# NeuralRevenant/RASSEngine

Hardware: AMD Instinct MI355X
Metric: queries/sec, exact cosine top-10 over N x 1024-d fp32 corpus in HBM (higher is better)
Workload: dtype f32; 1 GPU; 1000000 x 1024-d flat cosine top-10, 1 x MI355X, precomputed embeddings (BASELINE configs[1]); rows_per_gpu=1000000, rows_global=1000000, dim=1024, k=10, query_batch=32, corpus_dtype=f32, layout=tile16, mode=flat

## Files before the change

### include/rass_engine.h

```cpp
#ifndef RASS_ENGINE_H
#define RASS_ENGINE_H

#include <stddef.h>
#include <stdint.h>

#ifdef __cplusplus
extern "C" {
#endif

#define RASS_ABI_VERSION 1

typedef enum rass_status {
    RASS_OK = 0,
    RASS_ERR_INVALID = -1,
    RASS_ERR_HIP = -2,
    RASS_ERR_OOM = -3,
    RASS_ERR_NOT_FOUND = -4,
    RASS_ERR_UNSUPPORTED = -5,
    RASS_ERR_IO = -6
} rass_status;

typedef enum rass_dtype {
    RASS_F32 = 0,
    RASS_BF16 = 1,
// ... 183 lines not shown
                                     int64_t* d_out_ids, int64_t* d_n_buckets, int64_t* d_total_hits, int32_t* d_status);

int rass_index_rows_gram(rass_index_t* idx, const int64_t* rows, int n_lists, int list_len, float* out);
int rass_index_rows_gram_device(rass_index_t* idx, const int64_t* d_rows, int n_lists, int list_len, float* d_out);

int rass_index_search_mmr(rass_index_t* idx, const float* queries, int nq, int k, int fetch_k,
                          const float* lambda, const int32_t* q_filter, const int32_t* q_filter_mask,
                          float* out_scores, int64_t* out_ids, int32_t* out_rank);
int rass_index_search_mmr_device(rass_index_t* idx, const float* d_queries, int nq, int k, int fetch_k,
                                 const float* d_lambda, const int32_t* d_q_filter, const int32_t* d_q_filter_mask,
                                 int64_t id_base, float* d_out_scores, int64_t* d_out_ids, int32_t* d_out_rank);

#define RASS_PREFILTER_OFF 0
#define RASS_PREFILTER_BF16 1
#define RASS_PREFILTER_INT8 2
#define RASS_PREFILTER_INT8_EXACT 3
int rass_index_set_prefilter(rass_index_t* idx, int enable);
int rass_index_get_prefilter(const rass_index_t* idx);
int rass_index_certify_stats(rass_index_t* idx, int64_t* queries, int64_t* certified, int64_t* fallbacks, float* R, float* V);
int rass_index_candidates_exact_device(rass_index_t* idx, const float* d_queries, int nq, int k, const int32_t* d_q_filter,
                                       float* d_cand_scores, int64_t* d_cand_rows, float* d_tau, int32_t* d_certified);
int rass_index_sample_floor_device(rass_index_t* idx, const float* d_queries, int nq, int k, const int32_t* d_q_filter,
                                   int32_t* d_out_rows, float* d_out_scores);
int rass_index_candidates_device(rass_index_t* idx, const float* d_queries, int nq, const int32_t* d_q_filter,
                                 float* d_cand_scores, int64_t* d_cand_rows);

int rass_index_save(rass_index_t* idx, const char* path);
int rass_index_load(rass_engine_t* eng, const char* name, const char* path,
                    rass_index_t** out);

int rass_index_fill_synthetic(rass_index_t* idx, int64_t n, uint64_t seed,
                              int64_t row_id_base);


size_t rass_scan_workspace_bytes(int nq, int k);

int rass_pack_rows_f32(const float* d_in, int64_t in_stride, float* d_packed,
                       int64_t row_stride, int64_t first_row, int64_t n, int dim,
                       int normalize, void* stream);
int rass_unpack_rows_f32(const float* d_packed, int64_t row_stride,
                         int64_t first_row, int64_t n, int dim, float* d_out,
                         int64_t out_stride, void* stream);
int rass_gather_rows_f32(const float* d_packed, int64_t row_stride, int64_t n_rows,
                         const int64_t* d_row_ids, int64_t n, int dim, float* d_out,
                         int64_t out_stride, void* stream);
int rass_compact_plan(const int32_t* d_tags, int64_t n_rows, int64_t* d_new_row,
// ... 203 lines not shown
```

### rassengine_amd/_native.py

```python
from __future__ import annotations

import ctypes
import os
from typing import Optional

_HERE = os.path.dirname(os.path.abspath(__file__))
LIB_PATH = os.environ.get("RASS_HIP_LIB") or os.path.join(_HERE, "lib", "librass_hip.so")

RASS_OK = 0
RASS_MAX_K = 32
RASS_MAX_K_MULTIPASS = 4096
RASS_TAG_PATIENT_MASK = 0x00FFFFFF
RASS_TAG_DOCTYPE_SHIFT = 24
RASS_TAG_DOCTYPE_MASK = 0x7F000000
RASS_MAX_QBATCH = 32
RASS_MAX_DEVICE_BATCH = 4096
RASS_MAX_MMR_FETCH = 128
RASS_F32 = 0
RASS_BF16 = 1
RASS_QFILTER_NONE = -1
RASS_MAX_ATTRS = 8
RASS_ATTR_MISSING = -(1 << 31)
RASS_MAX_ATTR_CLAUSES = 64
RASS_ATTR_ALL, RASS_ATTR_ANY = 0, 1
# ... 103 lines not shown
    "rass_index_search_grouped_keys_device": (ctypes.c_int, [ctypes.c_void_p, ctypes.c_void_p, ctypes.c_int, ctypes.c_int, ctypes.c_void_p, ctypes.c_int64, ctypes.c_int32, ctypes.c_void_p, ctypes.c_int, ctypes.c_int64, ctypes.c_void_p, ctypes.c_void_p, ctypes.c_int64, ctypes.c_void_p, ctypes.c_void_p, ctypes.c_void_p, ctypes.c_void_p, ctypes.c_void_p]),
    "rass_index_aggregate_keys": (ctypes.c_int, [ctypes.c_void_p, ctypes.c_void_p, ctypes.c_int, ctypes.c_void_p, ctypes.c_int, ctypes.c_void_p, ctypes.c_int64, ctypes.c_int32, ctypes.c_void_p, ctypes.c_int, ctypes.c_int64, ctypes.c_void_p, ctypes.c_void_p, ctypes.c_void_p, ctypes.c_void_p, ctypes.c_void_p, ctypes.c_void_p, ctypes.c_void_p, ctypes.c_void_p]),
    "rass_index_aggregate_keys_device": (ctypes.c_int, [ctypes.c_void_p, ctypes.c_void_p, ctypes.c_int, ctypes.c_void_p, ctypes.c_int, ctypes.c_void_p, ctypes.c_int64, ctypes.c_int32, ctypes.c_void_p, ctypes.c_int, ctypes.c_int64, ctypes.c_void_p, ctypes.c_void_p, ctypes.c_int64, ctypes.c_void_p, ctypes.c_void_p, ctypes.c_void_p, ctypes.c_void_p, ctypes.c_void_p, ctypes.c_void_p, ctypes.c_void_p]),
    "rass_index_rows_gram": (ctypes.c_int, [ctypes.c_void_p, ctypes.c_void_p, ctypes.c_int, ctypes.c_int, ctypes.c_void_p]),
    "rass_index_rows_gram_device": (ctypes.c_int, [ctypes.c_void_p, ctypes.c_void_p, ctypes.c_int, ctypes.c_int,
                                                   ctypes.c_void_p]),
    "rass_index_search_mmr": (ctypes.c_int, [ctypes.c_void_p, ctypes.c_void_p, ctypes.c_int, ctypes.c_int, ctypes.c_int,
                                             ctypes.c_void_p, ctypes.c_void_p, ctypes.c_void_p, ctypes.c_void_p, ctypes.c_void_p,
                                             ctypes.c_void_p]),
    "rass_index_search_mmr_device": (ctypes.c_int, [ctypes.c_void_p, ctypes.c_void_p, ctypes.c_int, ctypes.c_int, ctypes.c_int,
                                                    ctypes.c_void_p, ctypes.c_void_p, ctypes.c_void_p, ctypes.c_int64,
                                                    ctypes.c_void_p, ctypes.c_void_p, ctypes.c_void_p]),
    "rass_index_set_prefilter": (ctypes.c_int, [ctypes.c_void_p, ctypes.c_int]),
    "rass_index_get_prefilter": (ctypes.c_int, [ctypes.c_void_p]),
    "rass_index_candidates_device": (ctypes.c_int, [ctypes.c_void_p, ctypes.c_void_p, ctypes.c_int, ctypes.c_void_p,
                                                    ctypes.c_void_p, ctypes.c_void_p]),
    "rass_index_certify_stats": (ctypes.c_int, [ctypes.c_void_p, ctypes.c_void_p, ctypes.c_void_p, ctypes.c_void_p,
                                                ctypes.c_void_p, ctypes.c_void_p]),
    "rass_index_candidates_exact_device": (ctypes.c_int, [ctypes.c_void_p, ctypes.c_void_p, ctypes.c_int, ctypes.c_int,
                                                          ctypes.c_void_p, ctypes.c_void_p, ctypes.c_void_p, ctypes.c_void_p,
                                                          ctypes.c_void_p]),
    "rass_index_sample_floor_device": (ctypes.c_int, [ctypes.c_void_p, ctypes.c_void_p, ctypes.c_int, ctypes.c_int,
                                                      ctypes.c_void_p, ctypes.c_void_p, ctypes.c_void_p]),
    "rass_index_save": (ctypes.c_int, [ctypes.c_void_p, ctypes.c_char_p]),
    "rass_index_load": (ctypes.c_int, [ctypes.c_void_p, ctypes.c_char_p, ctypes.c_char_p, c_void_pp]),
    "rass_index_fill_synthetic": (ctypes.c_int, [ctypes.c_void_p, ctypes.c_int64, ctypes.c_uint64,
                                                 ctypes.c_int64]),
    "rass_scan_workspace_bytes": (ctypes.c_size_t, [ctypes.c_int, ctypes.c_int]),
    "rass_scan_topk_f32": (ctypes.c_int, [ctypes.c_void_p, ctypes.c_int64, ctypes.c_int, ctypes.c_int64,
                                          ctypes.c_void_p, ctypes.c_void_p, ctypes.c_int, ctypes.c_void_p,
                                          ctypes.c_int, ctypes.c_int64, ctypes.c_void_p, ctypes.c_void_p,
                                          ctypes.c_void_p, ctypes.c_size_t, ctypes.c_void_p]),
    "rass_pack_rows_f32": (ctypes.c_int, [ctypes.c_void_p, ctypes.c_int64, ctypes.c_void_p, ctypes.c_int64,
                                          ctypes.c_int64, ctypes.c_int64, ctypes.c_int, ctypes.c_int,
                                          ctypes.c_void_p]),
    "rass_unpack_rows_f32": (ctypes.c_int, [ctypes.c_void_p, ctypes.c_int64, ctypes.c_int64, ctypes.c_int64,
                                            ctypes.c_int, ctypes.c_void_p, ctypes.c_int64, ctypes.c_void_p]),
    "rass_gather_rows_f32": (ctypes.c_int, [ctypes.c_void_p, ctypes.c_int64, ctypes.c_int64, ctypes.c_void_p, ctypes.c_int64,
                                            ctypes.c_int, ctypes.c_void_p, ctypes.c_int64, ctypes.c_void_p]),
    "rass_compact_plan": (ctypes.c_int, [ctypes.c_void_p, ctypes.c_int64, ctypes.c_void_p, ctypes.c_void_p, ctypes.c_void_p,
                                         ctypes.c_void_p, ctypes.c_size_t, ctypes.c_void_p]),
    "rass_compact_plan_workspace_bytes": (ctypes.c_size_t, [ctypes.c_int64]),
    "rass_compact_rows_f32": (ctypes.c_int, [ctypes.c_void_p, ctypes.c_void_p, ctypes.c_int64, ctypes.c_void_p, ctypes.c_int64,
                                             ctypes.c_int64, ctypes.c_void_p]),
    "rass_topk_merge": (ctypes.c_int, [ctypes.c_void_p, ctypes.c_void_p, ctypes.c_int, ctypes.c_int, ctypes.c_int,
                                       ctypes.c_void_p, ctypes.c_void_p, ctypes.c_void_p]),
# ... 167 lines not shown
```

### rassengine_amd/csrc/api_internal.h

```cpp
#pragma once

#include <hip/hip_runtime.h>
#include <stdint.h>
#include <stdio.h>
#include <stdlib.h>
#include <string.h>
#include <unistd.h>

#include <algorithm>
#include <atomic>
#include <condition_variable>
#include <map>
#include <mutex>
#include <new>
#include <string>
#include <type_traits>
#include <vector>

#include "../../include/rass_engine.h"
#include "kernels.h"

namespace rass {
namespace host {

// ... 76 lines not shown
struct ScratchView {
    float* q_padded;
    float* part_scores;
    int64_t* part_ids;
    unsigned short* q_bf16;
    float* cand_scores;
    int64_t* cand_ids;
    float* sample_best;
    size_t total;
};
ScratchView scratch_layout(unsigned char* base, int nq, int k);

struct BatchView {
    float* q_padded;
    float* part_scores;
    int64_t* part_ids;
    float* sample_best;
    unsigned char* q_small;
    float* cand_scores;
    int64_t* cand_rows;
    unsigned char* rep_qfrag;
    unsigned char* rep_part;
    int* rep_row;
    size_t total;
    size_t part_per_group;
    float* group_sample(int g) const { return sample_best + (int64_t)g * 32 * rass::kMaxSampleGroups; }
};
BatchView batch_layout(unsigned char* base, int groups, int grid, int k, int64_t stride, bool candidates = false);

struct CertView {
    float* q_padded;
    signed char* q8;
    rass::CertQInfo* qinfo;
    float* sample;
    float* list_s;
    int32_t* list_r;
    int32_t* list_n;
    float* list_floor;
    int64_t* cand_rows;
    float* rr_s;
    int64_t* rr_i;
    float* tau;
    int32_t *fail_idx, *fail_flag, *fail_n;
    float* fb_q;
    int32_t *fb_filter, *fb_mask;
    float* fb_s;
// ... 186 lines not shown
    float* d_pair_scores = nullptr;
    int64_t* d_pair_ids = nullptr;
    unsigned char* d_batch = nullptr;
    size_t batch_bytes = 0;
    unsigned char* d_allow_ws = nullptr;
    size_t allow_ws_bytes = 0;
};

namespace rass {
namespace host {

int set_device(const rass_engine* eng);
int index_reserve(rass_index* idx, int64_t need_rows);
void index_free_slabs(rass_index* idx);
int index_attr_ensure(rass_index* idx, int col);
int index_refresh_copies(rass_index* idx, int64_t first, int64_t n, hipStream_t st);

int scan_xcd_skew(int nq, int grid, int n_cus);
int64_t scan_sample_floor_min_share();
bool i8_sample_floor(int64_t rows, int grid);
enum { kBatchSampleGroups = 0, kBatchSampleF32 = 1, kBatchSampleRep = 2 };
int scan_batch_sample_mode();
bool scan_batch_pair();
bool ivf_batch_one_launch();

int scan_grid(int64_t tiles, int lists_kept_per_wg, int n_cus);

template <class F>
int timed_launch(rass_engine* eng, hipStream_t st, F&& launch, int extra_groups = 0) {
    const bool timed = eng && eng->ev_on && (size_t)(2 * eng->ev_used + 1) < eng->ev_pool.size();
    if (timed) HIP_TRY(hipEventRecord(eng->ev_pool[2 * eng->ev_used], st));
    const int rc = launch();
    if (rc != RASS_OK) return rc;
    if (timed) {
        HIP_TRY(hipEventRecord(eng->ev_pool[2 * eng->ev_used + 1], st));
        eng->ev_used += 1;
        eng->ev_extra += extra_groups;
    }
    return RASS_OK;
}

inline void as_sample(rass::ScanArgs& s) { s.xcd_skew = 0, s.sample_pass = true; }
inline void as_sample(rass::ScanBf16Args& s) { s.k = 1; }
inline void as_sample(rass::ScanI8Args& s) { s.k = 1; }
template <class Args>
int sample_prelaunch(Args& a, int grid, float* best, hipError_t (*launch)(const Args&, int, hipStream_t), hipStream_t st,
// ... 153 lines not shown
```

### rassengine_amd/csrc/api_scan.hip

```cpp

#include "api_internal.h"

namespace rass {
namespace host {


int scan_xcd_skew(int nq, int grid, int n_cus) {
    struct Skew {
        int b16 = 4, b32 = 0;
        Skew() {
            if (const char* e = getenv("RASS_SCAN_XCD_SKEW")) {
                int a = 0, b = 0;
                const int n = sscanf(e, "%d,%d", &a, &b);
                if (n == 1) b = a;
                if (n >= 1 && a >= 0 && b >= 0 && a <= 4096 && b <= 4096) b16 = a, b32 = b;
            }
        }
    };
    if (grid != n_cus || grid % 8 != 0) return 0;
    static const Skew skew;
    return nq <= 16 ? skew.b16 : skew.b32;
}

int64_t scan_sample_floor_min_share() {
// ... 5 lines not shown

bool i8_sample_floor(int64_t rows, int grid) {
    const char* e = getenv("RASS_I8_SAMPLE_FLOOR");
    const bool force = e && e[0] == 'f';
    if (e && !force && atoi(e) == 0) return false;
    return grid <= rass::kMaxSampleGroups && rows >= (int64_t)(force ? 2 : 8) * 64 * grid;
}

int scan_batch_sample_mode() {
    const char* e = getenv("RASS_SCAN_BATCH_SAMPLE");
    if (e && e[0] == 'g') return kBatchSampleGroups;
    if (e && e[0] == 'f') return kBatchSampleF32;
    return kBatchSampleRep;
}

bool scan_batch_pair() {
    static const bool on = [] {
        const char* e = getenv("RASS_SCAN_BATCH_PAIR");
        return !(e && e[0] == '0');
    }();
    return on;
}

bool ivf_batch_one_launch() {
    const char* e = getenv("RASS_IVF_BATCH_FINE");
    return !(e && e[0] == 'g');
}


int scan_grid(int64_t tiles, int lists_kept_per_wg, int n_cus) {
    int grid = (int)std::min<int64_t>(std::max<int64_t>(tiles, 1), std::min(n_cus, kMaxGrid));
    if ((int64_t)grid * lists_kept_per_wg > rass::kMergeMaxCandidates) grid = rass::kMergeMaxCandidates / lists_kept_per_wg;
    return grid;
}

ScratchView scratch_layout(unsigned char* base, int nq, int k) {
    Carver c{base};
    ScratchView L;
    L.q_padded = c.take<float>((size_t)RASS_MAX_QBATCH * kMaxStride * sizeof(float));
    L.part_scores = c.take<float>((size_t)kMaxGrid * nq * k * sizeof(float));
    L.part_ids = c.take<int64_t>((size_t)kMaxGrid * nq * k * sizeof(int64_t));
    L.q_bf16 = c.take<unsigned short>((size_t)RASS_MAX_QBATCH * kMaxStride * 2);
    L.cand_scores = c.take<float>((size_t)RASS_MAX_QBATCH * RASS_MAX_K * sizeof(float));
    L.cand_ids = c.take<int64_t>((size_t)RASS_MAX_QBATCH * RASS_MAX_K * sizeof(int64_t));
    L.sample_best = c.take<float>((size_t)rass::kMaxSampleGroups * 32 * sizeof(float));
    L.total = c.off;
    return L;
}

BatchView batch_layout(unsigned char* base, int groups, int grid, int k, int64_t stride, bool candidates) {
    Carver c{base};
    BatchView L;
    L.part_per_group = (size_t)grid * 32 * k;
    L.q_padded = c.take<float>((size_t)groups * 32 * stride * sizeof(float));
    L.part_scores = c.take<float>((size_t)groups * L.part_per_group * sizeof(float));
    L.part_ids = c.take<int64_t>((size_t)groups * L.part_per_group * sizeof(int64_t));
    L.sample_best = c.take<float>((size_t)groups * 32 * rass::kMaxSampleGroups * sizeof(float));
    L.q_small = candidates ? c.take<unsigned char>((size_t)groups * 32 * kMaxStride * 2) : nullptr;
    L.cand_scores = candidates ? c.take<float>((size_t)groups * 32 * k * sizeof(float)) : nullptr;
    L.cand_rows = candidates ? c.take<int64_t>((size_t)groups * 32 * k * sizeof(int64_t)) : nullptr;
    L.rep_qfrag = candidates ? nullptr : c.take<unsigned char>((size_t)groups * 32 * stride * 2);
    L.rep_part = candidates ? nullptr : c.take<unsigned char>((size_t)groups * 32 * rass::kMaxSampleGroups * 8);
    L.rep_row = candidates ? nullptr : c.take<int>((size_t)groups * 32 * 32 * sizeof(int));
    L.total = c.off;
    return L;
}

CertView cert_layout(unsigned char* base, int grid, int64_t stride, int64_t stride_i8, int dim) {
    Carver c{base};
    CertView L;
    const size_t Q = rass::kCertQ, slots = (size_t)grid * Q * rass::kCertWgCap;
    L.q_padded = c.take<float>(4 * Q * stride * sizeof(float));
    L.q8 = c.take<signed char>(2 * Q * stride_i8);
    L.qinfo = c.take<rass::CertQInfo>(Q * sizeof(rass::CertQInfo));
    L.sample = c.take<float>((size_t)rass::kMaxSampleGroups * Q * sizeof(float));
    L.list_s = c.take<float>(slots * sizeof(float));
    L.list_r = c.take<int32_t>(slots * sizeof(int32_t));
    L.list_n = c.take<int32_t>((size_t)grid * Q * sizeof(int32_t));
    L.list_floor = c.take<float>((size_t)grid * Q * sizeof(float));
    L.cand_rows = c.take<int64_t>(Q * rass::kCertC * sizeof(int64_t));
    L.rr_s = c.take<float>(Q * rass::kCertC * sizeof(float));
    L.rr_i = c.take<int64_t>(Q * rass::kCertC * sizeof(int64_t));
    L.tau = c.take<float>(Q * sizeof(float));
    L.fail_idx = c.take<int32_t>(Q * sizeof(int32_t));
    L.fail_flag = c.take<int32_t>(Q * sizeof(int32_t));
    L.fail_n = c.take<int32_t>(sizeof(int32_t));
// ... 394 lines not shown
```

### rassengine_amd/csrc/api_search.hip

```cpp

#include "api_internal.h"

namespace rass {
namespace host {

HostSlot* slot_acquire(rass_engine* eng) {
    std::unique_lock<std::mutex> lk(eng->slot_mu);
    for (;;) {
        for (HostSlot& sl : eng->slots)
            if (!sl.busy) {
                sl.busy = true;
                return &sl;
            }
        eng->slot_cv.wait(lk);
    }
}

void slot_release(rass_engine* eng, HostSlot* sl) {
    {
        std::lock_guard<std::mutex> lk(eng->slot_mu);
        sl->busy = false;
    }
    eng->slot_cv.notify_one();
}
// ... 126 lines not shown
        HIP_TRY(rass::launch_sample_rep(iv.corpus, iv.row_tag, stride, grid, L.q_padded, r.q_filter, nq, L.rep_qfrag, L.rep_part,
                                        L.rep_row, L.sample_best, st));
    } else if (one_sample) {
        rass::ScanArgs s = group_args(0);
        s.n_rows = (int)sample_rows;
        s.xcd_skew = 0;
        s.sample_pass = true;
        s.nq = 32;
        s.part_scores = L.sample_best;
        s.part_ids = nullptr;
        s.wgs_per_group = sample_wgs;
        s.q_group_stride = 32 * stride;
        s.part_group_stride = (int64_t)32 * rass::kMaxSampleGroups;
        s.nq_total = nq;
        HIP_TRY(rass::launch_scan_topk_f32(s, groups * sample_wgs, st));
    } else if (sample)
        for (int g = 0; g < groups; ++g) {
            rass::ScanArgs a = group_args(g);
            if (a.nq <= 16) continue;
            rc = sample_prelaunch(a, grid, L.group_sample(g), rass::launch_scan_topk_f32, st);
            if (rc != RASS_OK) return rc;
        }
    const bool pairs = scan_batch_pair() && rass::scan_pair_supported_stride(stride);
    for (int g = 0; g < groups; ++g) {
        rass::ScanArgs a = group_args(g);
        if (sample && a.nq > 16) {
            a.sample_best = L.group_sample(g);
            a.sample_groups = sample_wgs;
        }
        const bool pair = pairs && a.nq == RASS_MAX_QBATCH && (g + 2) * RASS_MAX_QBATCH <= nq;
        if (pair) {
            a.nq = 2 * RASS_MAX_QBATCH;
            a.q_group_stride = 32 * stride;
            a.part_group_stride = (int64_t)L.part_per_group;
            a.xcd_skew = scan_xcd_skew(a.nq, grid, eng->n_cus);
            rc = timed_launch(eng, st, [&] { return HIP_RC(rass::launch_scan_topk_f32_pair(a, grid, st)); }, 1);
            ++g;
        } else
            rc = timed_launch(eng, st, [&] { return HIP_RC(rass::launch_scan_topk_f32(a, grid, st)); });
        if (rc != RASS_OK) return rc;
    }
    const rass::MergeGroups mg = dense_groups(nq, (int64_t)L.part_per_group, gs, gi);
    HIP_TRY(rass::launch_merge_topk(L.part_scores, L.part_ids, grid, nq, k, r.out_scores, r.out_ids, st, iv.id_map, 0, 0, &mg));
    return RASS_OK;
}

int sample_floor_hook(rass_index* idx, const float* d_queries, int nq, int k, const int32_t* d_q_filter, int32_t* d_rows,
                      float* d_scores) {
    rass_engine* eng = idx->eng;
    hipStream_t st = eng->stream;
    const IndexView iv = index_view(idx, d_q_filter != nullptr, 0);
    const int64_t stride = idx->stride;
    if (idx->dtype != RASS_F32 || idx->prefilter || nq <= RASS_MAX_QBATCH || iv.rows <= 0 || iv.rows > kMaxScanRows ||
        stride > kNarrowStride || !rass::scan_supported_stride(stride))
        return fail(RASS_ERR_UNSUPPORTED, "not a fused fp32 batch");
    const BatchSamplePlan plan = batch_sample_plan(eng, iv.rows, stride, nq, k);
    if (!plan.rep) return fail(RASS_ERR_UNSUPPORTED, "this batch does not take the representatives' sample stage");
    const int groups = nq / RASS_MAX_QBATCH;
    int rc = grow_block(&eng->d_batch, &eng->batch_bytes, batch_layout(nullptr, groups, plan.grid, k, stride).total, st);
    if (rc != RASS_OK) return rc;
    const BatchView L = batch_layout(eng->d_batch, groups, plan.grid, k, stride);
    HIP_TRY(rass::launch_normalize_rows_f32(d_queries, idx->dim, L.q_padded, stride, nq, idx->dim, st, nq));
    HIP_TRY(rass::launch_sample_rep(iv.corpus, iv.row_tag, stride, plan.grid, L.q_padded, d_q_filter, nq, L.rep_qfrag, L.rep_part,
                                    L.rep_row, L.sample_best, st));
    HIP_TRY(hipMemcpyAsync(d_rows, L.rep_row, (size_t)nq * 32 * sizeof(int32_t), hipMemcpyDeviceToDevice, st));
    HIP_TRY(hipMemcpy2DAsync(d_scores, 32 * sizeof(float), L.sample_best, rass::kMaxSampleGroups * sizeof(float), 32 * sizeof(float),
                             (size_t)nq, hipMemcpyDeviceToDevice, st));
    return RASS_OK;
}

int prefilter_launch_batch(rass_index* idx, const FlatRequest& r, int64_t gs, int64_t gi) {
    rass_engine* eng = idx->eng;
    hipStream_t st = eng->stream;
    const int nq = r.nq;
    const IndexView iv = index_view(idx, r.q_filter != nullptr, r.id_base);
    const int64_t rows = iv.rows;
    const int64_t stride = idx->stride;
    const int kc = RASS_MAX_K;
    const int groups = (nq + RASS_MAX_QBATCH - 1) / RASS_MAX_QBATCH;
    const int grid = scan_grid((rows + 63) / 64, kc, eng->n_cus);
    int rc = grow_block(&eng->d_batch, &eng->batch_bytes, batch_layout(nullptr, groups, grid, kc, stride, true).total, st);
    if (rc != RASS_OK) return rc;
    const BatchView L = batch_layout(eng->d_batch, groups, grid, kc, stride, true);
    const int nq_pad = groups * 32;
    HIP_TRY(rass::launch_normalize_rows_f32(r.queries, idx->dim, L.q_padded, stride, nq, idx->dim, st, nq_pad));
    const bool i8 = idx->prefilter == 2;
    const int64_t qs_stride = i8 ? idx->stride_i8 : stride * 2;
// ... 222 lines not shown
    rass_engine* eng = idx->eng;
    std::lock_guard<std::mutex> lk(eng->mu);
    int rc = set_device(eng);
    if (rc != RASS_OK) return rc;
    if (idx->prefilter != 3 || idx->dtype != RASS_F32) return fail(RASS_ERR_UNSUPPORTED, "the index is not in prefilter mode 3");
    if (idx->rows.load(std::memory_order_acquire) <= 0) return fail(RASS_ERR_INVALID, "the index is empty");
    FlatRequest r;
    r.queries = d_queries, r.nq = nq, r.k = k, r.q_filter = d_q_filter;
    r.row_tag = index_view(idx, d_q_filter != nullptr).row_tag;
    r.cand_scores = d_cand_scores, r.cand_rows = d_cand_rows, r.tau = d_tau, r.certified = d_certified;
    return cert_launch(idx, r);
}

int rass_index_sample_floor_device(rass_index_t* idx, const float* d_queries, int nq, int k, const int32_t* d_q_filter,
                                   int32_t* d_out_rows, float* d_out_scores) {
    if (!idx || !d_queries || !d_out_rows || !d_out_scores) return fail(RASS_ERR_INVALID, "NULL argument");
    if (nq < 1 || nq > RASS_MAX_DEVICE_BATCH) return fail(RASS_ERR_INVALID, "nq must be in [1, RASS_MAX_DEVICE_BATCH]");
    if (int rc = check_k(k)) return rc;
    rass_engine* eng = idx->eng;
    std::lock_guard<std::mutex> lk(eng->mu);
    int rc = set_device(eng);
    if (rc != RASS_OK) return rc;
    return sample_floor_hook(idx, d_queries, nq, k, d_q_filter, d_out_rows, d_out_scores);
}

int rass_index_search_ex(rass_index_t* idx, const float* queries, int nq, int k, const int32_t* q_filter,
                         const int32_t* q_filter_mask, float* out_scores, int64_t* out_ids) {
    if (!idx || !out_scores || !out_ids) return fail(RASS_ERR_INVALID, "NULL argument");
    if (nq < 0 || (nq > 0 && !queries)) return fail(RASS_ERR_INVALID, "bad queries / nq");
    if (k < 1 || k > RASS_MAX_K_MULTIPASS) return fail(RASS_ERR_INVALID, "k must be in [1, RASS_MAX_K_MULTIPASS]");
    if (q_filter_mask && !q_filter) return fail(RASS_ERR_INVALID, "q_filter_mask without q_filter");
    return one_layout([&] { return idx->layout_epoch.load(std::memory_order_acquire); },
                      [&] { return search_ex_once(idx, queries, nq, k, q_filter, q_filter_mask, out_scores, out_ids); });
}

static int search_multi_once(rass_engine* eng, rass_index_t* const* idxs, const float* queries, int nq, int k,
                             const int32_t* q_filter, const int32_t* q_filter_mask, float* out_scores, int64_t* out_ids) {
    int rc = set_device(eng);
    if (rc != RASS_OK) return rc;
    const int dim = eng->dim;
    SlotGuard guard(eng);
    HostSlot* sl = guard.sl;
    const size_t item_bytes = 4 + 4 + 4 + 8 + 8;
    if (!sl->h_items) HIP_TRY(hipHostMalloc(&sl->h_items, (size_t)kMultiMaxItems * item_bytes, hipHostMallocDefault));
    int32_t* h_tile = static_cast<int32_t*>(sl->h_items);
    int32_t* h_rows = h_tile + kMultiMaxItems;
// ... 118 lines not shown
```

### rassengine_amd/csrc/kernels.h

```cpp
#pragma once

#include <hip/hip_runtime.h>
#include <stddef.h>
#include <stdint.h>

namespace rass {

constexpr int kMaxSampleGroups = 256;

struct ScanArgs {
    const float* corpus;
    const int32_t* row_tag;
    const float* q_padded;
    const int32_t* q_filter;
    const int32_t* q_filter_mask = nullptr;
    const float* q_after_score = nullptr;
    const int64_t* q_after_id = nullptr;
    float* part_scores;
    int64_t* part_ids;
    int64_t row_stride;
    int64_t id_base;
    int n_rows;
    int nq;
    int k;
    const int32_t* work_tile = nullptr;
    const int32_t* work_rows = nullptr;
    const uint32_t* work_mask = nullptr;
    const int32_t* n_work = nullptr;
    const float* const* work_base = nullptr;
    const int32_t* const* work_tags = nullptr;
    const float* sample_best = nullptr;
    int sample_groups = 0;
    bool sample_pass = false;
    int xcd_skew = 0;
    const int32_t* live_nq = nullptr;
    int wgs_per_group = 0;
    int64_t q_group_stride = 0, part_group_stride = 0;
    int64_t work_group_stride = 0;
    int nq_total = 0;
    const float* range_thr = nullptr;
    unsigned* range_count = nullptr;
    union {
        uint2* range_hits = nullptr;
        const int32_t* group_keys;
    };
    int range_cap = 0;
    unsigned long long* group_table = nullptr;
    unsigned* group_status = nullptr;
    int group_mask = 0, group_shift = 0, group_n = 0;
    int group_key_rows = 0;
    const uint32_t* allow = nullptr;
    int64_t allow_q_stride = 0;
    unsigned* count_table = nullptr;
};
static_assert(sizeof(ScanArgs) == 312 && offsetof(ScanArgs, range_hits) == 240 && offsetof(ScanArgs, group_keys) == 240 &&
                  offsetof(ScanArgs, range_cap) == 248 && offsetof(ScanArgs, group_n) == 280 &&
                  offsetof(ScanArgs, group_key_rows) == 284 && offsetof(ScanArgs, allow) == 288 &&
                  offsetof(ScanArgs, count_table) == 304,
              "ScanArgs grew or moved a field: every scan kernel's device code changes with it");
constexpr int kRangeCountStride = 32;
constexpr int kRangeMaxHits = 4096;

bool scan_supported_stride(int64_t row_stride);
hipError_t launch_scan_topk_f32(const ScanArgs& a, int grid, hipStream_t stream);
bool scan_pair_supported_stride(int64_t row_stride);
hipError_t launch_scan_topk_f32_pair(const ScanArgs& a, int grid, hipStream_t stream);

constexpr int kMergeMaxCandidates = 8192;
struct MergeGroups {
    int size = 0;
    int nq_total = 0;
    bool lists_are_dense = false;
    int64_t score_stride = 0, id_stride = 0, out_score_stride = 0, out_id_stride = 0;
};
hipError_t launch_merge_topk(const float* scores, const int64_t* ids, int n_lists, int nq, int k,
                             float* out_scores, int64_t* out_ids, hipStream_t stream,
                             const int64_t* id_map = nullptr, int64_t score_list_stride = 0,
                             int64_t id_list_stride = 0, const MergeGroups* groups = nullptr,
                             const int32_t* live_nq = nullptr);

hipError_t launch_range_finish(const unsigned* count, const uint2* hits, int nq, int cap, int64_t id_base, const int64_t* id_map,
                               float* out_scores, int64_t* out_ids, int64_t* total, hipStream_t stream);

constexpr int kGroupMaxK = 4096;
constexpr int kGroupMaxGroups = 1 << 20;
hipError_t launch_group_select(const unsigned long long* table, int nq, int n_groups, int k, int64_t id_base, const int64_t* id_map,
                               float* out_scores, int64_t* out_ids, int32_t* out_groups, int64_t* total, const unsigned* status,
                               int32_t* out_status, hipStream_t stream);
hipError_t launch_group_count_select(const unsigned* counts, const unsigned long long* best, int nq, int n_groups, int size, int64_t id_base,
// ... 63 lines not shown
    int k;
    int64_t id_base = 0;
    const int32_t* q_filter_mask = nullptr;
    const float* q_after_score = nullptr;
    const int64_t* q_after_id = nullptr;
    const int32_t* work_tile = nullptr;
    const int32_t* work_rows = nullptr;
    const uint32_t* work_mask = nullptr;
    const int32_t* n_work = nullptr;
    const float* sample_best = nullptr;
    int sample_groups = 0;
};
hipError_t launch_scan_bf16_topk(const ScanBf16Args& a, int grid, hipStream_t stream);
hipError_t launch_convert_tile16_bf16(const float* src, void* dst, int64_t stride, int64_t block0, int64_t block1,
                                      hipStream_t stream, int64_t src_block0 = -1, int64_t row_lo = 0,
                                      int64_t row_hi = -1);
hipError_t launch_unpack_rows_tile16b(const void* slab, int64_t stride, int64_t first_row, int64_t n, int dim,
                                      float* out, int64_t out_stride, hipStream_t stream);
hipError_t launch_queries_to_bf16(const float* src, void* dst, int64_t n, hipStream_t stream);
bool sample_rep_supported(int64_t stride, int grid);
hipError_t launch_sample_rep(const float* slab, const int32_t* row_tag, int64_t stride, int grid, const float* q_padded,
                             const int32_t* q_filter, int nq, void* q_frag, void* rep_part, int* rep_row, float* sample_best,
                             hipStream_t stream);
hipError_t launch_rerank_f32(const float* slab, int64_t stride, const float* q_padded, const int64_t* cand_rows, int nq,
                             int n_cand, int k, int64_t id_base, float* out_scores, int64_t* out_ids,
                             hipStream_t stream, int64_t out_scores_group_stride = 0, int64_t out_ids_group_stride = 0,
                             const int64_t* id_map = nullptr);

struct ScanI8Args {
    const signed char* corpus;
    const float* row_scale;
    const int32_t* row_tag;
    const signed char* q_i8;
    const int32_t* q_filter;
    float* part_scores;
    int64_t* part_ids;
    int64_t row_stride;
    int n_rows;
    int nq;
    int k;
    const float* sample_best = nullptr;
    int sample_groups = 0;
    const int32_t* q_filter_mask = nullptr;
    int wgs_per_group = 0;
    int64_t q_group_stride = 0, part_group_stride = 0;
    const int32_t* work_tile = nullptr;
// ... 159 lines not shown
```

### rassengine_amd/csrc/sample_rep.hip

```cpp

#include <hip/hip_runtime.h>
#include <limits.h>
#include <stdint.h>

#include "kernels.h"
#include "scan_core.h"
#include "exact_score.h"

namespace rass {

typedef __bf16 bf16x8 __attribute__((ext_vector_type(8)));
typedef __bf16 bf16x4 __attribute__((ext_vector_type(4)));

constexpr int kRepThreads = 512;
constexpr int kRepRows = 64;

__device__ __forceinline__ bf16x8 pack_bf16(const f32x4 a, const f32x4 b) {
    const bf16x4 lo = __builtin_convertvector(a, bf16x4), hi = __builtin_convertvector(b, bf16x4);
    return __builtin_shufflevector(lo, hi, 0, 1, 2, 3, 4, 5, 6, 7);
}

__device__ __forceinline__ void take_better(float& s, int& r, float os, int orow) {
    const bool take = (os > s) | ((os == s) & (orow < r));
    s = take ? os : s;
// ... 173 lines not shown
                             const int32_t* q_filter, int nq, void* q_frag, void* rep_part, int* rep_row, float* sample_best,
                             hipStream_t stream) {
    if (!sample_rep_supported(stride, grid) || nq < 32 || nq % 32 != 0) return hipErrorInvalidValue;
    bf16x8* const qf = static_cast<bf16x8*>(q_frag);
    int2* const part = static_cast<int2*>(rep_part);
    const int n_frag = (int)((int64_t)nq * stride / 8);
    hipLaunchKernelGGL(sample_queries_frag_kernel, dim3((n_frag + 255) / 256), dim3(256), 0, stream, q_padded, stride, qf, n_frag);
#define RASS_REP_CASE(C)                                                                                                      \
    case C:                                                                                                                   \
        hipLaunchKernelGGL(sample_rep_bf16_kernel<C>, dim3(grid), dim3(kRepThreads), 0, stream, slab, row_tag, qf, q_filter,  \
                           nq / 16, part);                                                                                    \
        hipLaunchKernelGGL(sample_rescore_f32_kernel<C>, dim3(256), dim3(256), 0, stream, slab, q_padded, part, grid, nq / 32, \
                           rep_row, sample_best);                                                                             \
        break;
    switch ((int)(stride >> 7)) {
        RASS_REP_CASE(1) RASS_REP_CASE(2) RASS_REP_CASE(3) RASS_REP_CASE(4)
        RASS_REP_CASE(5) RASS_REP_CASE(6) RASS_REP_CASE(7) RASS_REP_CASE(8)
        default: return hipErrorInvalidValue;
    }
#undef RASS_REP_CASE
    return hipGetLastError();
}

}
```

### rassengine_amd/engine.py

```python
from __future__ import annotations

import ctypes
import threading
from typing import Dict, Optional, Tuple

import numpy as np

from . import _native as N


def _np_ptr(a: Optional[np.ndarray]):
    return None if a is None else a.ctypes.data_as(ctypes.c_void_p)


def pack_allow(mask: np.ndarray) -> np.ndarray:
    m = np.asarray(mask, dtype=bool)
    if m.ndim not in (1, 2):
        raise ValueError(f"expected a boolean mask [n] or [nb, n], got shape {m.shape}")
    n = m.shape[-1]
    words = (n + 31) // 32
    padded = np.zeros(m.shape[:-1] + (words * 32,), dtype=bool)
    padded[..., :n] = m
    packed = np.packbits(padded, axis=-1, bitorder="little")
    return np.ascontiguousarray(packed).view("<u4").reshape(m.shape[:-1] + (words,)).astype(np.uint32, copy=False)
# ... 261 lines not shown
                                                           ctypes.c_void_p(f.data_ptr()) if f is not None else None,
                                                           ctypes.c_void_p(s.data_ptr()), ctypes.c_void_p(r.data_ptr()),
                                                           ctypes.c_void_p(tau.data_ptr()), ctypes.c_void_p(cert.data_ptr())))
        self.engine.synchronize()
        return s, r, tau, cert

    def sample_floor_device(self, d_queries, k: int, q_filter=None):
        import torch
        nq = int(d_queries.shape[0])
        assert d_queries.is_cuda and d_queries.dtype == torch.float32 and d_queries.is_contiguous() and d_queries.shape[1] == self.dim
        dev = d_queries.device
        rows = torch.empty((nq, 32), dtype=torch.int32, device=dev)
        scores = torch.empty((nq, 32), dtype=torch.float32, device=dev)
        f = None
        if q_filter is not None:
            f = torch.as_tensor(np.ascontiguousarray(q_filter, dtype=np.int32)).to(dev)
        torch.cuda.current_stream().synchronize()
        N.check("rass_index_sample_floor_device",
                self._L.rass_index_sample_floor_device(self._h, ctypes.c_void_p(d_queries.data_ptr()), nq, int(k),
                                                       ctypes.c_void_p(f.data_ptr()) if f is not None else None,
                                                       ctypes.c_void_p(rows.data_ptr()), ctypes.c_void_p(scores.data_ptr())))
        self.engine.synchronize()
        return rows, scores

    def candidates_device(self, d_queries, q_filter=None):
        import torch
        nq = int(d_queries.shape[0])
        assert d_queries.is_cuda and d_queries.dtype == torch.float32 and d_queries.is_contiguous() and d_queries.shape[1] == self.dim
        s = torch.empty((nq, 32), dtype=torch.float32, device=d_queries.device)
        r = torch.empty((nq, 32), dtype=torch.int64, device=d_queries.device)
        f = None
        if q_filter is not None:
            f = torch.as_tensor(np.ascontiguousarray(q_filter, dtype=np.int32)).to(d_queries.device)
        torch.cuda.current_stream().synchronize()
        N.check("rass_index_candidates_device",
                self._L.rass_index_candidates_device(self._h, ctypes.c_void_p(d_queries.data_ptr()), nq,
                                                     ctypes.c_void_p(f.data_ptr()) if f is not None else None,
                                                     ctypes.c_void_p(s.data_ptr()), ctypes.c_void_p(r.data_ptr())))
        self.engine.synchronize()
        return s, r

    def save(self, path: str) -> None:
        N.check("rass_index_save", self._L.rass_index_save(self._h, path.encode()))

    def _queries(self, queries) -> np.ndarray:
        q = np.ascontiguousarray(queries, dtype=np.float32)
# ... 690 lines not shown
```

Baseline: 59470 queries/s.

## Add persistent multi-pair step scan kernel with precomputed sample floors

Adds a persistent scan kernel that walks several 64-query pairs in one launch, wrapping tiles across pairs and reloading queries in-kernel, instead of one launch per pair. A new step_floors kernel derives per-query score floors from the sample pass by bitwise selection, and the scan uses them to reject candidates before top-k insertion. The aim is to cut launch overhead and tail idle time between pair launches and to reduce insertion work. In exchange it adds complexity and a floor-correctness dependency, and it only applies when the batch holds at least two pairs.

Measured after the change: 60200 queries/s (median of 6 runs). 1.2% higher.

```diff
diff --git a/include/rass_engine.h b/include/rass_engine.h
--- a/include/rass_engine.h
+++ b/include/rass_engine.h
@@ -229,6 +229,8 @@
                                        float* d_cand_scores, int64_t* d_cand_rows, float* d_tau, int32_t* d_certified);
 int rass_index_sample_floor_device(rass_index_t* idx, const float* d_queries, int nq, int k, const int32_t* d_q_filter,
                                    int32_t* d_out_rows, float* d_out_scores);
+int rass_index_step_floors_device(rass_index_t* idx, const float* d_queries, int nq, int k, const int32_t* d_q_filter,
+                                  float* d_out_floors);
 int rass_index_candidates_device(rass_index_t* idx, const float* d_queries, int nq, const int32_t* d_q_filter,
                                  float* d_cand_scores, int64_t* d_cand_rows);
 
diff --git a/rassengine_amd/_native.py b/rassengine_amd/_native.py
--- a/rassengine_amd/_native.py
+++ b/rassengine_amd/_native.py
@@ -149,6 +149,8 @@
                                                           ctypes.c_void_p]),
     "rass_index_sample_floor_device": (ctypes.c_int, [ctypes.c_void_p, ctypes.c_void_p, ctypes.c_int, ctypes.c_int,
                                                       ctypes.c_void_p, ctypes.c_void_p, ctypes.c_void_p]),
+    "rass_index_step_floors_device": (ctypes.c_int, [ctypes.c_void_p, ctypes.c_void_p, ctypes.c_int, ctypes.c_int,
+                                                     ctypes.c_void_p, ctypes.c_void_p]),
     "rass_index_save": (ctypes.c_int, [ctypes.c_void_p, ctypes.c_char_p]),
     "rass_index_load": (ctypes.c_int, [ctypes.c_void_p, ctypes.c_char_p, ctypes.c_char_p, c_void_pp]),
     "rass_index_fill_synthetic": (ctypes.c_int, [ctypes.c_void_p, ctypes.c_int64, ctypes.c_uint64,
diff --git a/rassengine_amd/csrc/api_internal.h b/rassengine_amd/csrc/api_internal.h
--- a/rassengine_amd/csrc/api_internal.h
+++ b/rassengine_amd/csrc/api_internal.h
@@ -122,6 +122,7 @@
     unsigned char* rep_qfrag;
     unsigned char* rep_part;
     int* rep_row;
+    float* step_floor;
     size_t total;
     size_t part_per_group;
     float* group_sample(int g) const { return sample_best + (int64_t)g * 32 * rass::kMaxSampleGroups; }
@@ -354,6 +355,7 @@
 enum { kBatchSampleGroups = 0, kBatchSampleF32 = 1, kBatchSampleRep = 2 };
 int scan_batch_sample_mode();
 bool scan_batch_pair();
+bool scan_batch_step();
 bool ivf_batch_one_launch();
 
 int scan_grid(int64_t tiles, int lists_kept_per_wg, int n_cus);
diff --git a/rassengine_amd/csrc/api_scan.hip b/rassengine_amd/csrc/api_scan.hip
--- a/rassengine_amd/csrc/api_scan.hip
+++ b/rassengine_amd/csrc/api_scan.hip
@@ -51,6 +51,11 @@
     return on;
 }
 
+bool scan_batch_step() {
+    const char* e = getenv("RASS_SCAN_BATCH_STEP");
+    return !(e && e[0] == '0');
+}
+
 bool ivf_batch_one_launch() {
     const char* e = getenv("RASS_IVF_BATCH_FINE");
     return !(e && e[0] == 'g');
@@ -91,6 +96,7 @@
     L.rep_qfrag = candidates ? nullptr : c.take<unsigned char>((size_t)groups * 32 * stride * 2);
     L.rep_part = candidates ? nullptr : c.take<unsigned char>((size_t)groups * 32 * rass::kMaxSampleGroups * 8);
     L.rep_row = candidates ? nullptr : c.take<int>((size_t)groups * 32 * 32 * sizeof(int));
+    L.step_floor = candidates ? nullptr : c.take<float>((size_t)groups * 32 * sizeof(float));
     L.total = c.off;
     return L;
 }
diff --git a/rassengine_amd/csrc/api_search.hip b/rassengine_amd/csrc/api_search.hip
--- a/rassengine_amd/csrc/api_search.hip
+++ b/rassengine_amd/csrc/api_search.hip
@@ -172,6 +172,9 @@
             if (rc != RASS_OK) return rc;
         }
     const bool pairs = scan_batch_pair() && rass::scan_pair_supported_stride(stride);
+    const int n_pairs = pairs ? nq / (2 * RASS_MAX_QBATCH) : 0;
+    const bool step = scan_batch_step() && n_pairs >= 2 && grid <= (rows + 31) / 32;
+    if (step && sample) HIP_TRY(rass::launch_step_floors(L.sample_best, sample_wgs, n_pairs * 64, k, L.step_floor, st));
     for (int g = 0; g < groups; ++g) {
         rass::ScanArgs a = group_args(g);
         if (sample && a.nq > 16) {
@@ -179,11 +182,20 @@
             a.sample_groups = sample_wgs;
         }
         const bool pair = pairs && a.nq == RASS_MAX_QBATCH && (g + 2) * RASS_MAX_QBATCH <= nq;
+        const int run = pair && step ? std::min(rass::kStepMaxPairs, n_pairs - g / 2) : 1;
         if (pair) {
             a.nq = 2 * RASS_MAX_QBATCH;
             a.q_group_stride = 32 * stride;
             a.part_group_stride = (int64_t)L.part_per_group;
             a.xcd_skew = scan_xcd_skew(a.nq, grid, eng->n_cus);
+        }
+        if (run >= 2) {
+            a.sample_best = nullptr, a.sample_groups = 0;
+            a.step_floors = sample ? L.step_floor + g * 32 : nullptr;
+            a.nq_total = 64 * run;
+            rc = timed_launch(eng, st, [&] { return HIP_RC(rass::launch_scan_topk_f32_step(a, grid, st)); }, 2 * run - 1);
+            g += 2 * run - 1;
+        } else if (pair) {
             rc = timed_launch(eng, st, [&] { return HIP_RC(rass::launch_scan_topk_f32_pair(a, grid, st)); }, 1);
             ++g;
         } else
@@ -196,7 +208,7 @@
 }
 
 int sample_floor_hook(rass_index* idx, const float* d_queries, int nq, int k, const int32_t* d_q_filter, int32_t* d_rows,
-                      float* d_scores) {
+                      float* d_scores, float* d_floors = nullptr) {
     rass_engine* eng = idx->eng;
     hipStream_t st = eng->stream;
     const IndexView iv = index_view(idx, d_q_filter != nullptr, 0);
@@ -213,6 +225,11 @@
     HIP_TRY(rass::launch_normalize_rows_f32(d_queries, idx->dim, L.q_padded, stride, nq, idx->dim, st, nq));
     HIP_TRY(rass::launch_sample_rep(iv.corpus, iv.row_tag, stride, plan.grid, L.q_padded, d_q_filter, nq, L.rep_qfrag, L.rep_part,
                                     L.rep_row, L.sample_best, st));
+    if (d_floors) {
+        HIP_TRY(rass::launch_step_floors(L.sample_best, 32, nq, k, L.step_floor, st));
+        HIP_TRY(hipMemcpyAsync(d_floors, L.step_floor, (size_t)nq * sizeof(float), hipMemcpyDeviceToDevice, st));
+        return RASS_OK;
+    }
     HIP_TRY(hipMemcpyAsync(d_rows, L.rep_row, (size_t)nq * 32 * sizeof(int32_t), hipMemcpyDeviceToDevice, st));
     HIP_TRY(hipMemcpy2DAsync(d_scores, 32 * sizeof(float), L.sample_best, rass::kMaxSampleGroups * sizeof(float), 32 * sizeof(float),
                              (size_t)nq, hipMemcpyDeviceToDevice, st));
@@ -481,6 +498,18 @@
     int rc = set_device(eng);
     if (rc != RASS_OK) return rc;
     return sample_floor_hook(idx, d_queries, nq, k, d_q_filter, d_out_rows, d_out_scores);
+}
+
+int rass_index_step_floors_device(rass_index_t* idx, const float* d_queries, int nq, int k, const int32_t* d_q_filter,
+                                  float* d_out_floors) {
+    if (!idx || !d_queries || !d_out_floors) return fail(RASS_ERR_INVALID, "NULL argument");
+    if (nq < 1 || nq > RASS_MAX_DEVICE_BATCH) return fail(RASS_ERR_INVALID, "nq must be in [1, RASS_MAX_DEVICE_BATCH]");
+    if (int rc = check_k(k)) return rc;
+    rass_engine* eng = idx->eng;
+    std::lock_guard<std::mutex> lk(eng->mu);
+    int rc = set_device(eng);
+    if (rc != RASS_OK) return rc;
+    return sample_floor_hook(idx, d_queries, nq, k, d_q_filter, nullptr, nullptr, d_out_floors);
 }
 
 int rass_index_search_ex(rass_index_t* idx, const float* queries, int nq, int k, const int32_t* q_filter,
diff --git a/rassengine_amd/csrc/kernels.h b/rassengine_amd/csrc/kernels.h
--- a/rassengine_amd/csrc/kernels.h
+++ b/rassengine_amd/csrc/kernels.h
@@ -38,7 +38,10 @@
     int64_t q_group_stride = 0, part_group_stride = 0;
     int64_t work_group_stride = 0;
     int nq_total = 0;
-    const float* range_thr = nullptr;
+    union {
+        const float* range_thr = nullptr;
+        const float* step_floors;
+    };
     unsigned* range_count = nullptr;
     union {
         uint2* range_hits = nullptr;
@@ -65,6 +68,8 @@
 hipError_t launch_scan_topk_f32(const ScanArgs& a, int grid, hipStream_t stream);
 bool scan_pair_supported_stride(int64_t row_stride);
 hipError_t launch_scan_topk_f32_pair(const ScanArgs& a, int grid, hipStream_t stream);
+constexpr int kStepMaxPairs = 16;
+hipError_t launch_scan_topk_f32_step(const ScanArgs& a, int grid, hipStream_t stream);
 
 constexpr int kMergeMaxCandidates = 8192;
 struct MergeGroups {
@@ -174,6 +179,7 @@
 hipError_t launch_sample_rep(const float* slab, const int32_t* row_tag, int64_t stride, int grid, const float* q_padded,
                              const int32_t* q_filter, int nq, void* q_frag, void* rep_part, int* rep_row, float* sample_best,
                              hipStream_t stream);
+hipError_t launch_step_floors(const float* sample_best, int sample_groups, int nq, int k, float* floors, hipStream_t stream);
 hipError_t launch_rerank_f32(const float* slab, int64_t stride, const float* q_padded, const int64_t* cand_rows, int nq,
                              int n_cand, int k, int64_t id_base, float* out_scores, int64_t* out_ids,
                              hipStream_t stream, int64_t out_scores_group_stride = 0, int64_t out_ids_group_stride = 0,
diff --git a/rassengine_amd/csrc/sample_rep.hip b/rassengine_amd/csrc/sample_rep.hip
--- a/rassengine_amd/csrc/sample_rep.hip
+++ b/rassengine_amd/csrc/sample_rep.hip
@@ -219,4 +219,34 @@
     return hipGetLastError();
 }
 
-}
+__global__ __launch_bounds__(256) void step_floors_kernel(const float* __restrict__ sample_best, int sample_groups, int nq, int k,
+                                                          float* __restrict__ floors) {
+    const int lane = lane_id();
+    const int q = blockIdx.x * 4 + (threadIdx.x >> 6);
+    if (q >= nq) return;
+    unsigned key[kMaxSampleGroups / 64];
+#pragma unroll
+    for (int j = 0; j < kMaxSampleGroups / 64; ++j) {
+        const int grp = lane + 64 * j;
+        const float v = grp < sample_groups ? sample_best[(int64_t)q * kMaxSampleGroups + grp] : -INFINITY;
+        key[j] = v == -INFINITY ? 0u : score_key(v);
+    }
+    unsigned T = 0;
+#pragma unroll 1
+    for (int b = 31; b >= 32 - kFloorBits; --b) {
+        const unsigned cand = T | (1u << b);
+        int c = 0;
+#pragma unroll
+        for (int j = 0; j < kMaxSampleGroups / 64; ++j) c += __popcll(__ballot(key[j] >= cand));
+        T = c >= k ? cand : T;
+    }
+    if (lane == 0) floors[q] = T ? key_score(T) : -INFINITY;
+}
+
+hipError_t launch_step_floors(const float* sample_best, int sample_groups, int nq, int k, float* floors, hipStream_t stream) {
+    if (sample_groups < 1 || sample_groups > kMaxSampleGroups || nq < 1 || k < 1) return hipErrorInvalidValue;
+    hipLaunchKernelGGL(step_floors_kernel, dim3((nq + 3) / 4), dim3(256), 0, stream, sample_best, sample_groups, nq, k, floors);
+    return hipGetLastError();
+}
+
+}
diff --git a/rassengine_amd/csrc/scan_step.hip b/rassengine_amd/csrc/scan_step.hip
--- /dev/null
+++ b/rassengine_amd/csrc/scan_step.hip
@@ -0,0 +1,230 @@
+#include <hip/hip_runtime.h>
+#include <stdint.h>
+
+#include "kernels.h"
+#include "scan_core.h"
+
+namespace rass {
+
+template <int CH>
+__global__ __launch_bounds__(kThreads, 2) void scan_topk_f32_step_kernel(ScanArgs p) {
+    constexpr int NT = 4, NQ = 64;
+    extern __shared__ __attribute__((aligned(16))) float lds[];
+
+    const int lane = lane_id();
+    const int wid = __builtin_amdgcn_readfirstlane(threadIdx.x >> 6);
+    const int m = lane & 15, g = lane >> 4;
+    const int G = gridDim.x, bid = blockIdx.x;
+    const int n_tiles = (p.n_rows + kTileRows - 1) / kTileRows;
+    const int pairs = p.nq_total / NQ;
+
+    f32x4 qf[NT][CH];
+    auto load_queries = [&](int pair, int ln) {
+        const int m = ln & 15, g = ln >> 4;
+        const float* qbase = p.q_padded + (int64_t)pair * 2 * p.q_group_stride + (int64_t)m * p.row_stride + wid * 16 * CH + 4 * g;
+#pragma unroll
+        for (int nt = 0; nt < NT; ++nt) {
+            const float* qn = qbase + (int64_t)(nt >> 1) * p.q_group_stride + (int64_t)(nt & 1) * 16 * p.row_stride;
+#pragma unroll
+            for (int j = 0; j < CH; ++j) qf[nt][j] = *reinterpret_cast<const f32x4*>(qn + 16 * j);
+        }
+    };
+    load_queries(0, lane);
+    const int voff_lane = wid * CH * 1024 + lane * 16;
+
+    TopList L[NT];
+    float tau[NT];
+    auto reset_lists = [&]() {
+#pragma unroll
+        for (int pq = 0; pq < NT; ++pq) {
+            L[pq].s = -INFINITY;
+            L[pq].i = 0x7fffffff;
+            tau[pq] = -INFINITY;
+        }
+    };
+    reset_lists();
+    __shared__ int sh_qfilt[NQ];
+    __shared__ float sh_floor[NQ];
+    __shared__ int sh_tags[2][32];
+    auto fill_query_state = [&](int pair, int ln) {
+        if (wid == 0) {
+            const int q = pair * NQ + ln;
+            sh_qfilt[ln] = p.q_filter != nullptr ? p.q_filter[q] : -1;
+            sh_floor[ln] = p.step_floors != nullptr ? p.step_floors[q] : -INFINITY;
+        }
+    };
+    fill_query_state(0, lane);
+    __syncthreads();
+
+    auto work = [&](int pair, int tile) {
+        int rows = p.n_rows - tile * kTileRows;
+        rows = rows > kTileRows ? kTileRows : rows;
+        WorkItem w;
+        w.tile = pair < pairs ? tile : 0;
+        w.rows = pair < pairs ? rows : 0;
+        w.mask = 0xffffffffu;
+        return w;
+    };
+
+    const int mt_step = 16 * (int)p.row_stride * 4;
+    HalfRegs<CH> R0, R1;
+    int tag;
+    int c_pair = 0, c_tile = bid;
+    WorkItem W0 = work(c_pair, c_tile);
+    {
+        const TileDesc d = make_tile_desc(p.corpus, p.row_stride, p.row_tag, W0);
+        tag = load_tag(d);
+        __builtin_amdgcn_sched_barrier(0);
+        issue_half_loads<CH>(R0, d, voff_lane, 0);
+        issue_half_loads<CH>(R1, d, voff_lane, mt_step);
+    }
+    __builtin_amdgcn_sched_barrier(0);
+
+    auto dump_half = [&](const f32x4 (&acc)[NT], int buf, int blk) {
+        float* P = lds + buf * (kWaves * NQ * kPitch);
+#pragma unroll
+        for (int nt = 0; nt < NT; ++nt)
+            *reinterpret_cast<f32x4*>(P + (wid * NQ + nt * 16 + m) * kPitch + blk * 16 + 4 * g) = acc[nt];
+    };
+    struct RankIn {
+        float pz[kWaves];
+        int tag, qfilt;
+        float floor;
+    };
+    RankIn RI[NT];
+    auto rank_load = [&](int buf, int pq) {
+        const float* P = lds + buf * (kWaves * NQ * kPitch);
+        const int r = lane & 31;
+        const int q = pq * 16 + (lane >> 5) * 8 + wid;
+        const float* src = P + q * kPitch + r;
+#pragma unroll
+        for (int wv = 0; wv < kWaves; ++wv) RI[pq].pz[wv] = src[wv * NQ * kPitch];
+        RI[pq].tag = sh_tags[buf][r];
+        RI[pq].qfilt = sh_qfilt[q];
+        RI[pq].floor = sh_floor[q];
+    };
+    auto rank_use = [&](const WorkItem& w, int pq) {
+        const int r = lane & 31;
+        const int row = w.tile * kTileRows + r;
+        const RankIn& in = RI[pq];
+        float s = in.pz[0];
+#pragma unroll
+        for (int wv = 1; wv < kWaves; ++wv) s += in.pz[wv];
+        const bool ok = (r < w.rows) & (in.tag != -1) & ((in.qfilt < 0) | (in.qfilt == in.tag)) & (s >= in.floor);
+        s = ok ? s : -INFINITY;
+        insert_candidates(L[pq], tau[pq], s, row, p.k);
+    };
+    auto write_lists = [&](int pair, int ln) {
+        const int lpos = ln & 31;
+#pragma unroll
+        for (int pq = 0; pq < NT; ++pq) {
+            const int ql = (pq & 1) * 16 + (ln >> 5) * 8 + wid;
+            if (lpos < p.k) {
+                const int64_t o = (int64_t)(pair * 2 + (pq >> 1)) * p.part_group_stride + ((int64_t)bid * 32 + ql) * p.k + lpos;
+                const bool filled = L[pq].i != 0x7fffffff;
+                p.part_scores[o] = filled ? L[pq].s : -INFINITY;
+                p.part_ids[o] = filled ? (p.id_base + (int64_t)L[pq].i) : (int64_t)-1;
+            }
+        }
+    };
+
+    auto slot_of = [](int part) { return (part * 2 * CH) / NT + (2 * CH > NT ? 1 : 0); };
+    WorkItem Pw{0, 0, 0u};
+    int cur = 0;
+    for (;;) {
+        f32x4 acc[NT];
+        if (wid == 0 && lane < 32) sh_tags[cur][lane] = tag;
+        const WorkItem Wc = W0;
+        int n_tile = c_tile + G, n_pair = c_pair;
+        {
+            const bool wrap = n_tile >= n_tiles;
+            n_tile = wrap ? n_tile - n_tiles : n_tile;
+            n_pair = wrap ? n_pair + 1 : n_pair;
+        }
+        const WorkItem Wn = work(n_pair, n_tile);
+        const TileDesc dn = make_tile_desc(p.corpus, p.row_stride, p.row_tag, Wn);
+        tag = load_tag(dn);
+        auto load_prev = [&](int slot) {
+#pragma unroll
+            for (int part = 0; part < NT; ++part)
+                if (slot_of(part) == slot) rank_load(cur ^ 1, part);
+        };
+        auto rank_prev = [&](int slot) {
+#pragma unroll
+            for (int part = 0; part < NT; ++part)
+                if (slot_of(part) == slot) rank_use(Pw, part);
+        };
+        multiply_and_refill_half<CH, NT>(R0, qf, acc, dn, voff_lane, 0, [&](int j) { load_prev(j); },
+                                         [&](int j) { rank_prev(j); });
+        dump_half(acc, cur, 0);
+        multiply_and_refill_half<CH, NT>(R1, qf, acc, dn, voff_lane, mt_step, [&](int j) { load_prev(CH + j); },
+                                         [&](int j) { rank_prev(CH + j); });
+        dump_half(acc, cur, 1);
+        W0 = Wn;
+        Pw = Wc;
+        __syncthreads();
+        cur ^= 1;
+        c_tile = n_tile;
+        if (__builtin_expect(n_pair != c_pair, 0)) {
+#pragma unroll
+            for (int pq = 0; pq < NT; ++pq) {
+                rank_load(cur ^ 1, pq);
+                rank_use(Pw, pq);
+            }
+            int ln = lane;
+            asm volatile("" : "+v"(ln));
+            write_lists(c_pair, ln);
+            if (n_pair >= pairs) break;
+            reset_lists();
+            Pw.rows = 0;
+            c_pair = n_pair;
+            load_queries(n_pair, ln);
+            __syncthreads();
+            fill_query_state(n_pair, ln);
+            __syncthreads();
+#pragma unroll
+            for (int nt = 0; nt < NT; ++nt)
+#pragma unroll
+                for (int j = 0; j < CH; ++j) asm volatile("" : "+v"(qf[nt][j]));
+        }
+    }
+}
+
+template <int CH>
+static hipError_t launch_step_variant(const ScanArgs& a, int grid, hipStream_t stream) {
+    constexpr size_t lds_bytes = (size_t)2 * kWaves * 64 * kPitch * sizeof(float);
+    static bool attr_set = false;
+    if (!attr_set) {
+        hipError_t e = hipFuncSetAttribute(reinterpret_cast<const void*>(&scan_topk_f32_step_kernel<CH>),
+                                           hipFuncAttributeMaxDynamicSharedMemorySize, (int)lds_bytes);
+        if (e != hipSuccess) return e;
+        attr_set = true;
+    }
+    hipLaunchKernelGGL((scan_topk_f32_step_kernel<CH>), dim3(grid), dim3(kThreads), lds_bytes, stream, a);
+    return hipGetLastError();
+}
+
+hipError_t launch_scan_topk_f32_step(const ScanArgs& a, int grid, hipStream_t stream) {
+    if (!scan_pair_supported_stride(a.row_stride)) return hipErrorInvalidValue;
+    const int pairs = a.nq_total / 64;
+    if (a.nq != 64 || a.nq_total != 64 * pairs || pairs < 1 || pairs > kStepMaxPairs || a.q_group_stride <= 0 ||
+        a.part_group_stride <= 0)
+        return hipErrorInvalidValue;
+    if (grid < 1 || grid > (a.n_rows + kTileRows - 1) / kTileRows) return hipErrorInvalidValue;
+    if (a.q_filter_mask || a.q_after_score || a.q_after_id || a.work_tile || a.work_base || a.sample_pass || a.live_nq ||
+        a.wgs_per_group || a.sample_best)
+        return hipErrorInvalidValue;
+    switch ((int)(a.row_stride / 128)) {
+        case 1: return launch_step_variant<1>(a, grid, stream);
+        case 2: return launch_step_variant<2>(a, grid, stream);
+        case 3: return launch_step_variant<3>(a, grid, stream);
+        case 4: return launch_step_variant<4>(a, grid, stream);
+        case 5: return launch_step_variant<5>(a, grid, stream);
+        case 6: return launch_step_variant<6>(a, grid, stream);
+        case 7: return launch_step_variant<7>(a, grid, stream);
+        case 8: return launch_step_variant<8>(a, grid, stream);
+        default: return hipErrorInvalidValue;
+    }
+}
+
+}
diff --git a/rassengine_amd/engine.py b/rassengine_amd/engine.py
--- a/rassengine_amd/engine.py
+++ b/rassengine_amd/engine.py
@@ -307,6 +307,23 @@
                                                        ctypes.c_void_p(rows.data_ptr()), ctypes.c_void_p(scores.data_ptr())))
         self.engine.synchronize()
         return rows, scores
+
+    def step_floors_device(self, d_queries, k: int, q_filter=None):
+        import torch
+        nq = int(d_queries.shape[0])
+        assert d_queries.is_cuda and d_queries.dtype == torch.float32 and d_queries.is_contiguous() and d_queries.shape[1] == self.dim
+        dev = d_queries.device
+        floors = torch.empty((nq,), dtype=torch.float32, device=dev)
+        f = None
+        if q_filter is not None:
+            f = torch.as_tensor(np.ascontiguousarray(q_filter, dtype=np.int32)).to(dev)
+        torch.cuda.current_stream().synchronize()
+        N.check("rass_index_step_floors_device",
+                self._L.rass_index_step_floors_device(self._h, ctypes.c_void_p(d_queries.data_ptr()), nq, int(k),
+                                                      ctypes.c_void_p(f.data_ptr()) if f is not None else None,
+                                                      ctypes.c_void_p(floors.data_ptr())))
+        self.engine.synchronize()
+        return floors
 
     def candidates_device(self, d_queries, q_filter=None):
         import torch
```
